# Nikhil-AI-Labs/image-super-resolution-2

Hardware: AMD Instinct MI355X
Metric: output MPix/s at x4 SR (256->1024) (higher is better)
Workload: dtype bf16 (bf16 MFMA operands, fp32 accumulate, fp32 activations in HBM)

## Files before the change

### image-super-resolution-2_amd/csrc/conv_gemm_bf16.hip

```cpp
#include "ff_common.h"

typedef __bf16 bf16x8 __attribute__((ext_vector_type(8)));
typedef __bf16 bf16x4 __attribute__((ext_vector_type(4)));

struct ConvBfParams {
  const float* in;
  const __bf16* w_hi;
  const __bf16* w_lo;
  const float* bias;
  const float* mul;
  const float* res;
  const float* kmul;
  float* out;
  int B, H, W, Cin, ldi;
  int Ho, Wo, Cout, ldo, ldr;
  int KH, KW, sy, sx, py, px;
  int K, Kp, M;
  int Cp;
  int act;
  float alpha;
  int shuffle;
  int vec_out;
  int gate;
};

template <int BM, int BN, int WM, int WN, bool VEC4, int NTERMS, int BKB>
__global__ __launch_bounds__(WM * WN * 64) void conv_igemm_bf16_kernel(ConvBfParams p) {
  constexpr int ROWB = BKB * 4 + 16, PLB = BKB * 2;
  constexpr int KQ = BKB / 4, QB = BKB / 8;
  constexpr int NT = WM * WN * 64;
  constexpr int TM = BM / WM, TN = BN / WN;
  constexpr int MI = TM / 32, NI = TN / 32;
  constexpr int RPP = NT / KQ;
  constexpr int AQ = BM / RPP;
  constexpr int BI = (BN * 2 * QB + NT - 1) / NT;
  static_assert(BM % RPP == 0, "A staging must tile the rows");
  extern __shared__ __attribute__((aligned(16))) unsigned char smem[];
  unsigned char* As = smem;
  unsigned char* Bs = smem + 2 * BM * ROWB;

  const int tid = threadIdx.x;
  const int lane = tid & 63, wid = tid >> 6;
  const int l31 = lane & 31, hh = lane >> 5;
  const int wr = wid / WN, wc = wid % WN;

  const int mtiles = (p.M + BM - 1) / BM, ntiles = (p.Cout + BN - 1) / BN;
  const int L = ff_xcd_remap(blockIdx.x, mtiles * ntiles);
  const int m0 = (L / ntiles) * BM, n0 = (L % ntiles) * BN;

  const int srow = tid / KQ, kq = tid % KQ;
  int a_b[AQ], a_iy[AQ], a_ix[AQ];
  bool a_ok[AQ];
#pragma unroll
  for (int i = 0; i < AQ; ++i) {
    const int m = m0 + srow + RPP * i;
    a_ok[i] = m < p.M;
    const int mm = a_ok[i] ? m : 0;
    const int ox = mm % p.Wo, t2 = mm / p.Wo;
    const int oy = t2 % p.Ho;
    a_b[i] = t2 / p.Ho;
    a_iy[i] = oy * p.sy - p.py;
    a_ix[i] = ox * p.sx - p.px;
  }
  const bool is1x1 = (p.KH == 1 && p.KW == 1);

  f32x4 ra[AQ];
  uint4 rb[BI];

  auto load_chunk = [&](int k0) {
    if (VEC4) {
      int ky = 0, kx = 0, ci;
      bool kok;
      if (p.Cp > 0) {
        const int tap = k0 / p.Cp;
        ci = k0 - tap * p.Cp + 4 * kq;
        kok = ci < p.Cin;
        ky = tap / p.KW;
        kx = tap - ky * p.KW;
      } else {
        const int k = k0 + 4 * kq;
        kok = k < p.K;
        ci = k;
        if (!is1x1 && kok) {
          const int tap = k / p.Cin;
          ci = k - tap * p.Cin;
          ky = tap / p.KW;
          kx = tap - ky * p.KW;
        }
      }
#pragma unroll
      for (int i = 0; i < AQ; ++i) {
        const int iy = a_iy[i] + ky, ix = a_ix[i] + kx;
        f32x4 v = {0.f, 0.f, 0.f, 0.f};
        if (kok && a_ok[i] && (unsigned)iy < (unsigned)p.H && (unsigned)ix < (unsigned)p.W)
          v = *reinterpret_cast<const f32x4*>(p.in + ((long long)(a_b[i] * p.H + iy) * p.W + ix) * p.ldi + ci);
        ra[i] = v;
      }
      if (p.kmul && kok) {
        const f32x4 km = *reinterpret_cast<const f32x4*>(p.kmul + ci);
#pragma unroll
        for (int i = 0; i < AQ; ++i) ra[i] *= km;
      }
    } else {
#pragma unroll
      for (int e = 0; e < 4; ++e) {
        const int k = k0 + 4 * kq + e;
        const bool kok = k < p.K;
        int ky = 0, kx = 0, ci = k;
// ... 17 lines not shown
    for (int j = 0; j < BI; ++j) {
      const int id = tid + NT * j;
      const int plane = id / (BN * QB), rem = id % (BN * QB);
      const int r = rem / QB, q = rem % QB;
      uint4 v = {0u, 0u, 0u, 0u};
      if (id < BN * 2 * QB && (NTERMS == 3 || plane == 0) && n0 + r < p.Cout) {
        const __bf16* src = (plane ? p.w_lo : p.w_hi) + (long long)(n0 + r) * p.Kp + k0 + 8 * q;
        v = *reinterpret_cast<const uint4*>(src);
      }
      rb[j] = v;
    }
  };

  auto store_chunk = [&](int buf) {
#pragma unroll
    for (int i = 0; i < AQ; ++i) {
      bf16x4 hi, lo;
#pragma unroll
      for (int e = 0; e < 4; ++e) {
        const float f = ra[i][e];
        const __bf16 h = (__bf16)f;
        hi[e] = h;
        lo[e] = (__bf16)(f - (float)h);
      }
      unsigned char* dst = As + (size_t)(buf * BM + srow + RPP * i) * ROWB + kq * 8;
      *reinterpret_cast<bf16x4*>(dst) = hi;
      if (NTERMS >= 2) *reinterpret_cast<bf16x4*>(dst + PLB) = lo;
    }
#pragma unroll
    for (int j = 0; j < BI; ++j) {
      const int id = tid + NT * j;
      const int plane = id / (BN * QB), rem = id % (BN * QB);
      const int r = rem / QB, q = rem % QB;
      if (id < BN * 2 * QB && (NTERMS == 3 || plane == 0))
        *reinterpret_cast<uint4*>(Bs + (size_t)(buf * BN + r) * ROWB + plane * PLB + q * 16) = rb[j];
    }
  };

  f32x16 acc[MI][NI];
#pragma unroll
  for (int i = 0; i < MI; ++i)
#pragma unroll
    for (int j = 0; j < NI; ++j)
#pragma unroll
      for (int r = 0; r < 16; ++r) acc[i][j][r] = 0.f;

  const int nchunks = p.Kp / BKB;
  load_chunk(0);
  store_chunk(0);
  __syncthreads();

  for (int c = 0; c < nchunks; ++c) {
    const int buf = c & 1;
    if (c + 1 < nchunks) load_chunk((c + 1) * BKB);
#pragma unroll
    for (int s = 0; s < BKB / 16; ++s) {
      bf16x8 ah[MI], al[MI], bh[NI], bl[NI];
#pragma unroll
      for (int i = 0; i < MI; ++i) {
        const unsigned char* ap = As + (size_t)(buf * BM + wr * TM + i * 32 + l31) * ROWB + 32 * s + 16 * hh;
        ah[i] = *reinterpret_cast<const bf16x8*>(ap);
        if (NTERMS >= 2) al[i] = *reinterpret_cast<const bf16x8*>(ap + PLB);
      }
#pragma unroll
      for (int j = 0; j < NI; ++j) {
        const unsigned char* bp = Bs + (size_t)(buf * BN + wc * TN + j * 32 + l31) * ROWB + 32 * s + 16 * hh;
        bh[j] = *reinterpret_cast<const bf16x8*>(bp);
        if (NTERMS == 3) bl[j] = *reinterpret_cast<const bf16x8*>(bp + PLB);
      }
#pragma unroll
      for (int i = 0; i < MI; ++i)
#pragma unroll
        for (int j = 0; j < NI; ++j) {
          if (NTERMS == 3) acc[i][j] = __builtin_amdgcn_mfma_f32_32x32x16_bf16(ah[i], bl[j], acc[i][j], 0, 0, 0);
          if (NTERMS >= 2) acc[i][j] = __builtin_amdgcn_mfma_f32_32x32x16_bf16(al[i], bh[j], acc[i][j], 0, 0, 0);
          acc[i][j] = __builtin_amdgcn_mfma_f32_32x32x16_bf16(ah[i], bh[j], acc[i][j], 0, 0, 0);
        }
    }
    if (c + 1 < nchunks) store_chunk(buf ^ 1);
    __syncthreads();
  }

  auto epilogue = [&](auto ACTC) {
    constexpr int ACT = decltype(ACTC)::value;
    const bool has_res = p.res != nullptr;
    if (p.gate) {
      float* tr = reinterpret_cast<float*>(smem) + wid * (32 * 36);
      const int grow = lane >> 2, seg = lane & 3;
#pragma unroll
      for (int j = 0; j < NI; ++j) {
        const int n = n0 + wc * TN + j * 32 + l31;
        const float bv = (p.bias && n < p.Cout) ? p.bias[n] : 0.f;
        const int nq = (n0 + wc * TN + j * 32) / 2 + 4 * seg;
        const bool nqok = nq < p.Cout / 2;
#pragma unroll
        for (int i = 0; i < MI; ++i) {
          const int mb = m0 + wr * TM + i * 32;
#pragma unroll
          for (int r = 0; r < 16; ++r) tr[((r & 3) + 8 * (r >> 2) + 4 * hh) * 36 + l31] = acc[i][j][r] + bv;
#pragma unroll
          for (int pass = 0; pass < 2; ++pass) {
            const int row = grow + 16 * pass;
            const f32x4 a = *reinterpret_cast<const f32x4*>(tr + row * 36 + 8 * seg);
            const f32x4 b2 = *reinterpret_cast<const f32x4*>(tr + row * 36 + 8 * seg + 4);
            const f32x4 o = {a[0] * a[1], a[2] * a[3], b2[0] * b2[1], b2[2] * b2[3]};
            const int m = mb + row;
            if (nqok && m < p.M) *reinterpret_cast<f32x4*>(p.out + (long long)m * p.ldo + nq) = o;
          }
        }
      }
      return;
    }
    if (p.vec_out) {
      float* tr = reinterpret_cast<float*>(smem) + wid * (32 * 36);
      const int tq = lane >> 3, q4 = 4 * (lane & 7);
#pragma unroll
      for (int j = 0; j < NI; ++j) {
        const int n = n0 + wc * TN + j * 32 + l31;
        const int nc = n < p.Cout ? n : 0;
        const float bv = p.bias ? p.bias[nc] : 0.f;
        const float mv = (p.mul ? p.mul[nc] : 1.f) * p.alpha;
        const int nq = n0 + wc * TN + j * 32 + q4;
        const bool nqok = nq < p.Cout;
#pragma unroll
        for (int i = 0; i < MI; ++i) {
          const int mb = m0 + wr * TM + i * 32;
          f32x4 rq[4];
          long long oo[4];
          bool ok[4];
#pragma unroll
          for (int k = 0; k < 4; ++k) {
            const int m = mb + tq + 8 * k;
            ok[k] = nqok && m < p.M;
            oo[k] = ok[k] ? (long long)m * p.ldo + nq : 0;
            f32x4 r0 = {0.f, 0.f, 0.f, 0.f};
            if (has_res) { const f32x4 u = *reinterpret_cast<const f32x4*>(p.res + (ok[k] ? (long long)m * p.ldr + nq : 0)); r0 = ok[k] ? u : r0; }
            rq[k] = r0;
          }
#pragma unroll
          for (int r = 0; r < 16; ++r)
            tr[((r & 3) + 8 * (r >> 2) + 4 * hh) * 36 + l31] = ff_act_c<ACT, true>(acc[i][j][r] + bv) * mv;
          f32x4 ov[4];
#pragma unroll
          for (int k = 0; k < 4; ++k) ov[k] = *reinterpret_cast<const f32x4*>(tr + (tq + 8 * k) * 36 + q4) + rq[k];
          if (nqok && mb + 32 <= p.M) {
#pragma unroll
            for (int k = 0; k < 4; ++k) *reinterpret_cast<f32x4*>(p.out + oo[k]) = ov[k];
          } else {
#pragma unroll
            for (int k = 0; k < 4; ++k)
              if (ok[k]) *reinterpret_cast<f32x4*>(p.out + oo[k]) = ov[k];
          }
        }
      }
      return;
    }
#pragma unroll
    for (int j = 0; j < NI; ++j) {
      const int n = n0 + wc * TN + j * 32 + l31;
      if (n >= p.Cout) continue;
      const float bv = p.bias ? p.bias[n] : 0.f;
      const float mv = (p.mul ? p.mul[n] : 1.f) * p.alpha;
#pragma unroll
      for (int i = 0; i < MI; ++i) {
        long long oidx[16];
        float rv[16];
        const int mb = m0 + wr * TM + i * 32 + 4 * hh;
        if (p.shuffle == 2) {
#pragma unroll
          for (int r = 0; r < 16; ++r) {
            const int m = mb + (r & 3) + 8 * (r >> 2);
            const int mm = m < p.M ? m : 0;
            const int ox = mm % p.Wo, t2 = mm / p.Wo;
            const int oy = t2 % p.Ho, b = t2 / p.Ho;
            const int co = n >> 2, dy = (n >> 1) & 1, dx = n & 1;
            const long long pix = ((long long)(b * 2 * p.Ho + 2 * oy + dy) * (2 * p.Wo) + 2 * ox + dx);
            oidx[r] = pix * p.ldo + co;
            rv[r] = has_res ? p.res[pix * p.ldr + co] : 0.f;
          }
        } else {
#pragma unroll
          for (int r = 0; r < 16; ++r) {
            const int m = mb + (r & 3) + 8 * (r >> 2);
            const int mm = m < p.M ? m : 0;
            oidx[r] = (long long)mm * p.ldo + n;
            rv[r] = has_res ? p.res[(long long)mm * p.ldr + n] : 0.f;
          }
        }
        if (mb + 28 < p.M) {
#pragma unroll
          for (int r = 0; r < 16; ++r) p.out[oidx[r]] = ff_act_c<ACT, true>(acc[i][j][r] + bv) * mv + rv[r];
        } else {
#pragma unroll
          for (int r = 0; r < 16; ++r) {
            const int m = mb + (r & 3) + 8 * (r >> 2);
            if (m < p.M) p.out[oidx[r]] = ff_act_c<ACT, true>(acc[i][j][r] + bv) * mv + rv[r];
          }
        }
      }
    }
  };
  FF_DISPATCH_ACT(p.act, epilogue)
}

template <int BM, int BN, int WM, int WN, int NT, int BKB = 32>
static int launch_bf(const ConvBfParams& p, bool vec4, hipStream_t st) {
  const int mt = ff_cdiv(p.M, BM), nt = ff_cdiv(p.Cout, BN);
  constexpr size_t lds = (size_t)2 * (BM + BN) * (BKB * 4 + 16);
  static_assert(lds <= 160 * 1024 && lds >= (size_t)WM * WN * 32 * 36 * 4, "LDS budget (staging ring; the epilogue patch reuses it)");
  dim3 grid((unsigned)(mt * nt)), block(WM * WN * 64);
  if (lds > 64 * 1024) {
    static bool attr_set[2] = {false, false};
    if (!attr_set[vec4 ? 1 : 0]) {
      hipError_t e = vec4 ? hipFuncSetAttribute(reinterpret_cast<const void*>(&conv_igemm_bf16_kernel<BM, BN, WM, WN, true, NT, BKB>),
                                                hipFuncAttributeMaxDynamicSharedMemorySize, (int)lds)
                          : hipFuncSetAttribute(reinterpret_cast<const void*>(&conv_igemm_bf16_kernel<BM, BN, WM, WN, false, NT, BKB>),
                                                hipFuncAttributeMaxDynamicSharedMemorySize, (int)lds);
      if (e != hipSuccess) { ff_set_error("ff_conv2d_bf16s: cannot raise dynamic LDS to %zu: %s", lds, hipGetErrorString(e)); return FF_ERR_LAUNCH; }
      attr_set[vec4 ? 1 : 0] = true;
    }
  }
  if (vec4)
    hipLaunchKernelGGL((conv_igemm_bf16_kernel<BM, BN, WM, WN, true, NT, BKB>), grid, block, lds, st, p);
  else
    hipLaunchKernelGGL((conv_igemm_bf16_kernel<BM, BN, WM, WN, false, NT, BKB>), grid, block, lds, st, p);
  FF_LAUNCH_CHECK("ff_conv2d_bf16s");
  return FF_OK;
}

template <int NT>
static int dispatch_bf(const ConvBfParams& p, bool vec4, int cfg, hipStream_t st) {
  switch (cfg) {
    case 1: return launch_bf<128, 128, 2, 2, NT>(p, vec4, st);
    case 2: return launch_bf<128, 64, 2, 2, NT>(p, vec4, st);
    case 3: return launch_bf<256, 32, 4, 1, NT>(p, vec4, st);
    case 4: return launch_bf<256, 192, 4, 2, NT>(p, vec4, st);
    case 5: return launch_bf<128, 128, 2, 4, NT>(p, vec4, st);
    case 6: return launch_bf<256, 128, 4, 2, NT>(p, vec4, st);
    case 7: return launch_bf<128, 64, 4, 2, NT>(p, vec4, st);
    case 8: return launch_bf<128, 128, 2, 4, NT, 64>(p, vec4, st);
    case 9: return launch_bf<128, 64, 4, 2, NT, 64>(p, vec4, st);
    default: ff_set_error("ff_conv2d_bf16s: bad tile_hint %d", cfg); return FF_ERR_ARG;
  }
}

extern "C" int ff_conv2d_bf16s(const float* in, const void* w_hi, const void* w_lo, int Kp, int Cp, const float* bias,
                               const float* mul, const float* res, float* out, int B, int H, int W, int Cin, int ldi,
                               int Ho, int Wo, int Cout, int ldo, int ldr, int KH, int KW, int sy, int sx, int py, int px,
                               int act, float alpha, int shuffle, int nterms, int tile_hint, const float* kmul, void* stream) {
  FF_CHECK_ARG(in && w_hi && out, "ff_conv2d_bf16s: null pointer");
  FF_CHECK_ARG(!kmul || (KH == 1 && KW == 1 && Cin % 4 == 0 && (((uintptr_t)kmul) & 15) == 0), "ff_conv2d_bf16s: kmul needs a 1x1 kernel, Cin %% 4 == 0 and a 16-byte aligned vector");
  FF_CHECK_ARG(nterms >= 1 && nterms <= 3 && (nterms < 3 || w_lo), "ff_conv2d_bf16s: nterms must be 1..3 (3 needs w_lo)");
  FF_CHECK_ARG(B > 0 && H > 0 && W > 0 && Cin > 0 && Cout > 0 && Ho > 0 && Wo > 0, "ff_conv2d_bf16s: bad dims");
  FF_CHECK_ARG(ldi >= Cin, "ff_conv2d_bf16s: ldi %d < Cin %d", ldi, Cin);
  FF_CHECK_ARG(KH > 0 && KW > 0 && sy > 0 && sx > 0 && py >= 0 && px >= 0, "ff_conv2d_bf16s: bad kernel geometry");
  FF_CHECK_ARG(Kp % 32 == 0 && Kp >= KH * KW * Cin, "ff_conv2d_bf16s: Kp must be K rounded up to 32");
  FF_CHECK_ARG(Cp == 0 || (Cp % 32 == 0 && Cp >= Cin && Kp == KH * KW * Cp), "ff_conv2d_bf16s: TAP layout needs Kp == taps * Cp, Cp = ceil32(Cin)");
  FF_CHECK_ARG((((uintptr_t)w_hi) & 15) == 0 && (!w_lo || (((uintptr_t)w_lo) & 15) == 0), "ff_conv2d_bf16s: weight planes must be 16-byte aligned");
  FF_CHECK_ARG(shuffle == 0 || shuffle == 1 || shuffle == 2, "ff_conv2d_bf16s: shuffle must be 0, 1 (SimpleGate pair product) or 2 (PixelShuffle)");
  FF_CHECK_ARG(shuffle != 2 || Cout % 4 == 0, "ff_conv2d_bf16s: shuffle needs Cout %% 4 == 0");
  FF_CHECK_ARG(shuffle != 1 || (Cout % 8 == 0 && !res && !mul && act == 0 && alpha == 1.f && ldo % 4 == 0 && (((uintptr_t)out) & 15) == 0),
               "ff_conv2d_bf16s: the pair-product epilogue needs Cout %% 8 == 0, no residual / scale / activation and 16-byte aligned output rows");
  FF_CHECK_ARG(ldo >= (shuffle == 2 ? Cout / 4 : shuffle == 1 ? Cout / 2 : Cout), "ff_conv2d_bf16s: ldo too small");
  FF_CHECK_ARG(!res || ldr >= (shuffle ? Cout / 4 : Cout), "ff_conv2d_bf16s: ldr too small");
  FF_CHECK_ARG((long long)B * Ho * Wo < (1LL << 31), "ff_conv2d_bf16s: M overflows int");
  ConvBfParams p;
  p.in = in; p.w_hi = (const __bf16*)w_hi; p.w_lo = (const __bf16*)w_lo; p.bias = bias; p.mul = mul; p.res = res; p.out = out;
  p.kmul = kmul; p.gate = shuffle == 1 ? 1 : 0;
  p.B = B; p.H = H; p.W = W; p.Cin = Cin; p.ldi = ldi;
  p.Ho = Ho; p.Wo = Wo; p.Cout = Cout; p.ldo = ldo; p.ldr = ldr;
  p.KH = KH; p.KW = KW; p.sy = sy; p.sx = sx; p.py = py; p.px = px;
  p.K = KH * KW * Cin; p.Kp = Kp; p.Cp = Cp; p.M = B * Ho * Wo;
  p.act = act; p.alpha = alpha; p.shuffle = shuffle;
  p.vec_out = shuffle == 0 && Cout % 4 == 0 && ldo % 4 == 0 && (((uintptr_t)out) & 15) == 0 &&
              (!res || (ldr % 4 == 0 && (((uintptr_t)res) & 15) == 0));
  const bool vec4 = (Cin % 4 == 0) && (ldi % 4 == 0) && (((uintptr_t)in & 15) == 0);
  FF_CHECK_ARG(Cp == 0 || vec4, "ff_conv2d_bf16s: TAP layout needs Cin %% 4 == 0 and 16-byte aligned rows");
  FF_CHECK_ARG(!kmul || vec4, "ff_conv2d_bf16s: kmul needs 16-byte aligned input rows");
  hipStream_t st = (hipStream_t)stream;
  int cfg = tile_hint;
  if (cfg <= 0) {
    const int r192 = Cout % 192, r128 = Cout % 128;
    if (Cout <= 32) cfg = 3;
    else if (Cout <= 64) cfg = 7;
    else if (r128 == 0) cfg = 5;
    else if (vec4 && p.M >= 256 * 64 && (r192 == 0 || r192 > 128) && (Cout <= 192 || p.K >= 320)) cfg = 4;
    else if (Cout > 256 || (Cout > 128 && p.K >= 512)) cfg = 5;
    else cfg = 7;
  }
  const bool k64 = Kp % 64 == 0 && (Cp == 0 || Cp % 64 == 0) && vec4;
  if (cfg >= 8 && !k64) cfg = cfg == 8 ? 5 : 7;
  switch (nterms) {
    case 1: return dispatch_bf<1>(p, vec4, cfg, st);
    case 2: return dispatch_bf<2>(p, vec4, cfg, st);
    default: return dispatch_bf<3>(p, vec4, cfg, st);
  }
}

__global__ __launch_bounds__(256) void split_bf16_kernel(const float* __restrict__ w, int N, int K, int Kp, int Cin, int Cp,
                                                         __bf16* __restrict__ hi, __bf16* __restrict__ lo) {
  const long long total = (long long)N * Kp;
  for (long long i = (long long)blockIdx.x * 256 + threadIdx.x; i < total; i += (long long)gridDim.x * 256) {
    const int kp = (int)(i % Kp);
    const long long n = i / Kp;
    int k = kp;
    bool ok = kp < K;
    if (Cp > 0) { const int tap = kp / Cp, ci = kp - tap * Cp; ok = ci < Cin; k = tap * Cin + ci; }
    const float f = ok ? w[n * K + k] : 0.f;
    const __bf16 h = (__bf16)f;
    hi[i] = h;
    if (lo) lo[i] = (__bf16)(f - (float)h);
  }
}

extern "C" int ff_split_bf16(const float* w, int N, int K, int Kp, int Cin, int Cp, void* hi, void* lo, void* stream) {
  FF_CHECK_ARG(w && hi && N > 0 && K > 0 && Kp % 32 == 0 && Kp >= K, "ff_split_bf16: bad args");
  FF_CHECK_ARG(Cp == 0 || (Cin > 0 && K % Cin == 0 && Cp % 32 == 0 && Cp >= Cin && Kp == (K / Cin) * Cp), "ff_split_bf16: bad TAP layout");
  long long nb = ((long long)N * Kp + 255) / 256;
  if (nb > 4096) nb = 4096;
  hipLaunchKernelGGL(split_bf16_kernel, dim3((unsigned)nb), dim3(256), 0, (hipStream_t)stream, w, N, K, Kp, Cin, Cp, (__bf16*)hi, (__bf16*)lo);
  FF_LAUNCH_CHECK("ff_split_bf16");
  return FF_OK;
}
```

### image-super-resolution-2_amd/ops.py

```python
from __future__ import annotations

from typing import Dict, Optional, Tuple

import torch

from . import lib as _lib

ACT = {None: 0, "none": 0, "gelu": 1, "relu": 2, "lrelu": 3, "sigmoid": 4}
T = torch.Tensor

_PROF = None
_META = [0.0, 0.0]


def _note(flops: float = 0.0, nbytes: float = 0.0):
    _META[0] += flops
    _META[1] += nbytes


def _numel(*ts) -> float:
    return float(sum(t.numel() * (t.element_size() / 4.0) for t in ts if t is not None))


def _instrument(fn):
# ... 297 lines not shown
    elif tuple(out.shape) != oshape:
        raise _lib.FFError(f"conv2d: out shape {tuple(out.shape)} != {oshape}")
    out_bf16 = out.dtype == torch.bfloat16
    op, ldo, *_ = _nhwc(out, "conv2d.out|bf16ok" if out_bf16 else "conv2d.out")
    halo_ok = (_HALO and _GEMM_MODE in ("bf16x3", "bf16") and (KH, KW) == (3, 3) and tuple(stride) == (1, 1) and tuple(pad) == (1, 1)
               and not dynamic_w and Cin >= 32 and Cin % 4 == 0 and ldi % 4 == 0 and xp % 16 == 0
               and (Cout <= 64 or Cin >= 128 or 128 < Cout <= 192 or _HALO_ALL) and H * W >= 1024 and xp != op and B * H * W * ldi < 2 ** 31)
    if (in_bf16 or out_bf16) and not (halo_ok and _GEMM_MODE == "bf16" and shuffle == 0 and res is None):
        raise _lib.FFError("conv2d: bf16 input / output rows exist for the LDS-resident 3x3 kernel in plain-bf16 mode only")
    rp, ldr = None, 0
    if res is not None:
        if tuple(res.shape) != oshape:
            raise _lib.FFError(f"conv2d: res shape {tuple(res.shape)} != {oshape}")
        rp, ldr, *_ = _nhwc(res, "conv2d.res")
    if (_SMALL and _GEMM_MODE != "f32" and (KH, KW) == (3, 3) and tuple(stride) == (1, 1) and tuple(pad) == (1, 1) and Cout <= 16
            and Cin * (1 if Cout == 1 else (4 if Cout <= 4 else 16)) <= 128 and shuffle == 0 and mul is None and not dynamic_w and H * W >= 4096 and xp != op):
        from . import prep as _prep
        ws = PREPARED.get(w, "small", lambda: _prep.pack_conv3x3_small(w, Cin))
        _lib.check(_L().ff_conv3x3_small(xp, ldi, ws.data_ptr(), ws.shape[2], _ptr(bias), rp, ldr, op, ldo, B, H, W, Cin, Cout, ACT[act],
                                         float(alpha), _stream()))
    elif _GEMM_MODE == "f32":
        _lib.check(_L().ff_conv2d(xp, w.data_ptr(), _ptr(bias), _ptr(mul), rp, op, B, H, W, Cin, ldi, Ho, Wo, Cout, ldo, ldr,
                                  KH, KW, stride[0], stride[1], pad[0], pad[1], ACT[act], float(alpha), shuffle, tile_hint,
                                  _stream()))
    elif (_HALO and _GEMM_MODE in ("bf16x3", "bf16") and (KH, KW) == (3, 3) and tuple(stride) == (1, 1) and tuple(pad) == (1, 1)
          and not dynamic_w and Cin >= 32 and Cin % 4 == 0 and ldi % 4 == 0 and xp % 16 == 0
          and (Cout <= 64 or Cin >= 128 or 128 < Cout <= 192 or _HALO_ALL)
          and H * W >= 1024 and xp != op and B * H * W * ldi < 2 ** 31):
        from . import prep as _prep

        nt_ = _nterms()

        def _mk_halo():
            bn = _prep.halo_bn(Cout)
            return (_prep.pack_conv3x3_halo(w, Cin, bn, nt_), bn)
        img = PREPARED.get(w, "halo" if nt_ == 3 else "halo1", _mk_halo)
        part = None
        if want_pool and B == 1 and shuffle == 0 and Cout <= img[1]:
            prow = int(_L().ff_conv3x3_halo_pool_rows(B, H, W, Cout, img[1], nt_))
            part = torch.empty((prow, img[1]), device=x.device, dtype=torch.float32)
        _lib.check(_L().ff_conv3x3_halo(xp, ldi, img[0].data_ptr(), img[1], _ptr(bias), _ptr(mul), rp, ldr, op, ldo, B, H, W,
                                        Cin, Cout, ACT[act], float(alpha), shuffle, _ptr(part), _nterms(),
                                        (1 if in_bf16 else 0) | (2 if out_bf16 else 0), _stream()))
        if part is not None:
            pp = PoolPartials(part, Cout, 1.0 / float(H * W))
            _note(2.0 * B * Ho * Wo * Cout * KH * KW * Cin, 4.0 * (_numel(x, w, out, res)))
            return out, (pp if want_pool == "partials" else pp.mean())
    else:
        aligned = (ldi % 4 == 0) and (xp % 16 == 0)
        hi, lo, Kp, Cp, _ = _split_weight(w, dynamic_w, Cin if aligned else 0)
        _lib.check(_L().ff_conv2d_bf16s(xp, hi.data_ptr(), lo.data_ptr() if lo is not None else None, Kp, Cp, _ptr(bias), _ptr(mul),
                                        rp, op, B, H, W, Cin, ldi, Ho, Wo, Cout, ldo, ldr, KH, KW, stride[0], stride[1],
                                        pad[0], pad[1], ACT[act], float(alpha), shuffle, GEMM_MODES[_GEMM_MODE], tile_hint,
                                        None, _stream()))
    _note(2.0 * B * Ho * Wo * Cout * KH * KW * Cin, 4.0 * (_numel(x, w, out, res)))
    if want_pool:
        return out, pool_mean(out)
    return out


def cab_fused(x: T, w1: T, b1: T, w2: T, b2: T, partials: bool = False):
    if _GEMM_MODE != "bf16":
        raise _lib.FFError("cab_fused exists for the plain-bf16 contraction mode only")
    xp, ldi, B, H, W, Cin = _nhwc(x, "cab_fused.x")
    Cmid, Cout = w1.shape[0], w2.shape[0]
    if B != 1 or w1.shape[1] != 9 * Cin or w2.shape[1] != 9 * Cmid:
        raise _lib.FFError("cab_fused: expects one image and packed 3x3 weights [Cmid, 9*Cin], [Cout, 9*Cmid]")
    from . import prep as _prep
    i1 = PREPARED.get(w1, "cab1", lambda: _prep.pack_conv3x3_halo(w1, Cin, 64, 1))
    i2 = PREPARED.get(w2, "cab2", lambda: _prep.pack_conv3x3_halo(w2, Cmid, 192, 1))
    out = empty_rows((1, H, W, Cout), x.device)
    op, ldo, *_ = _nhwc(out, "cab_fused.out")
    prow = int(_L().ff_cab_fused_pool_rows(H, W))
    part = torch.empty((prow, 192), device=x.device, dtype=torch.float32)
    _lib.check(_L().ff_cab_fused(xp, ldi, i1.data_ptr(), b1.data_ptr(), i2.data_ptr(), b2.data_ptr(), op, ldo, H, W, Cin, Cmid, Cout,
                                 part.data_ptr(), _stream()))
    pp = PoolPartials(part, Cout, 1.0 / float(H * W))
    _note(2.0 * H * W * 9 * (Cmid * Cin + Cout * Cmid), 4.0 * H * W * (Cin + Cout))
    return out, (pp if partials else pp.mean())


def linear(x: T, w: T, bias: Optional[T] = None, *, act=None, res: Optional[T] = None, mul: Optional[T] = None,
           alpha: float = 1.0, out: Optional[T] = None, dynamic_w: bool = False, kmul: Optional[T] = None,
           gate_pairs: bool = False) -> T:
    xp, ldi, rows, K = rows_view(x, "linear.x")
    N = w.shape[0]
    if w.dim() != 2 or w.shape[1] != K or not w.is_contiguous():
        raise _lib.FFError(f"linear: weight must be [N, {K}], got {tuple(w.shape)}")
    if (kmul is not None or gate_pairs) and _GEMM_MODE == "f32":
        raise _lib.FFError("linear: kmul / gate_pairs exist in the split-bf16 kernels only")
    No = N // 2 if gate_pairs else N
    oshape = tuple(x.shape[:-1]) + (No,)
    if out is None:
        out = empty_rows(oshape, x.device)
    op, ldo, orows, oc = rows_view(out, "linear.out")
    if orows != rows or oc != No:
        raise _lib.FFError("linear: out shape mismatch")
    rp, ldr = None, 0
    if res is not None:
        rp, ldr, rrows, rc = rows_view(res, "linear.res")
        if rrows != rows or rc != N:
            raise _lib.FFError("linear: res shape mismatch")
    if _GEMM_MODE == "f32":
        _lib.check(_L().ff_conv2d(xp, w.data_ptr(), _ptr(bias), _ptr(mul), rp, op, 1, 1, rows, K, ldi, 1, rows, N, ldo, ldr,
                                  1, 1, 1, 1, 0, 0, ACT[act], float(alpha), 0, 0, _stream()))
    else:
        aligned = (ldi % 4 == 0) and (xp % 16 == 0)
        hi, lo, Kp, Cp, _ = _split_weight(w, dynamic_w, K if aligned else 0)
        if kmul is not None and (kmul.numel() != K or not kmul.is_contiguous()):
            raise _lib.FFError(f"linear: kmul must be a contiguous [{K}] vector")
        _lib.check(_L().ff_conv2d_bf16s(xp, hi.data_ptr(), lo.data_ptr() if lo is not None else None, Kp, Cp, _ptr(bias), _ptr(mul),
                                        rp, op, 1, 1, rows, K, ldi, 1, rows, N, ldo, ldr, 1, 1, 1, 1, 0, 0, ACT[act],
                                        float(alpha), 1 if gate_pairs else 0, GEMM_MODES[_GEMM_MODE], 0, _ptr(kmul), _stream()))
    _note(2.0 * rows * N * K, 4.0 * (rows * K + N * K + rows * No * (2 if res is not None else 1)))
    return out


def window_attn(qkv: T, out: T, biasT: T, *, q_off: int, k_off: int, v_off: int, o_off: int, H: int, W: int, Hp: int,
                Wp: int, win: Tuple[int, int], kwin: Tuple[int, int], shift: Tuple[int, int], use_mask: bool, heads: int,
                d: int, scale: float, rel_table: Optional[T] = None) -> T:
    qp, ldq, B, h_, w_, _ = _nhwc(qkv, "window_attn.qkv")
    op, ldo, *_ = _nhwc(out, "window_attn.out")
    if (h_, w_) != (H, W) or tuple(out.shape[:3]) != (B, H, W):
        raise _lib.FFError("window_attn: qkv/out spatial dims mismatch")
    nk = kwin[0] * kwin[1]
    if tuple(biasT.shape) != (heads, nk, 256) or not biasT.is_contiguous():
        raise _lib.FFError(f"window_attn: biasT must be [{heads},{nk},256]")
    if q_off + heads * d > qkv.shape[-1] or k_off + heads * d > qkv.shape[-1] or v_off + heads * d > qkv.shape[-1] \
            or o_off + heads * d > out.shape[-1]:
        raise _lib.FFError("window_attn: channel offsets out of range")
    if _GEMM_MODE == "f32":
        _lib.check(_L().ff_window_attn(qp, ldq, q_off, k_off, v_off, op, ldo, o_off, biasT.data_ptr(), B, H, W, Hp, Wp, win[0],
                                       win[1], kwin[0], kwin[1], shift[0], shift[1], int(use_mask), heads, d, float(scale),
                                       _stream()))
    else:
        relp = None
        if rel_table is not None and tuple(kwin) != tuple(win):
            n = (win[0] + kwin[0] - 1) * (win[1] + kwin[1] - 1)
            if tuple(rel_table.shape) != (heads, n) or not rel_table.is_contiguous() or kwin[1] % 8 or tuple(shift) != (0, 0):
                raise _lib.FFError(f"window_attn: overlapping-window rel_table must be [heads, {n}] (prep.pack_rel_overlap), kw % 8 == 0, no shift")
            relp = rel_table.data_ptr()
        elif rel_table is not None and tuple(kwin) == tuple(win) and win[1] & (win[1] - 1) == 0 and win[1] >= 8:
            if tuple(rel_table.shape) != (heads, (2 * win[0] - 1) * (2 * win[1] - 1)) or not rel_table.is_contiguous():
                raise _lib.FFError("window_attn: rel_table must be [heads, (2wh-1)*(2ww-1)]")
            relp = rel_table.data_ptr()
        from . import prep as _prep
        bq = PREPARED.get(biasT, "quad", lambda: _prep.quad_bias(biasT))
        _lib.check(_L().ff_window_attn_bf16s(qp, ldq, q_off, k_off, v_off, op, ldo, o_off, bq.data_ptr(), B, H, W, Hp, Wp,
                                             win[0], win[1], kwin[0], kwin[1], shift[0], shift[1], int(use_mask), heads, d,
                                             float(scale), 1 if _GEMM_MODE == "bf16" else 3, relp, _stream()))
    nwin = B * (Hp // win[0]) * (Wp // win[1])
    _note(4.0 * nwin * heads * 256 * nk * d, 4.0 * (4.0 * B * H * W * heads * d + heads * nk * 256))
    return out


def ocab_attn(qkv: T, out: T, rel_rotated: T, *, q_off: int, k_off: int, v_off: int, o_off: int = 0, H: int, W: int, heads: int, d: int,
              ws: int, ows: int, scale: float) -> T:
    if _GEMM_MODE != "bf16":
        raise _lib.FFError("ocab_attn exists for the plain-bf16 contraction mode only")
    qp, ldq, B, h_, w_, _ = _nhwc(qkv, "ocab_attn.qkv")
    out_bf16 = out.dtype == torch.bfloat16
    op, ldo, *_ = _nhwc(out, "ocab_attn.out|bf16ok" if out_bf16 else "ocab_attn.out")
    if (h_, w_) != (H, W) or tuple(out.shape[:3]) != (B, H, W) or tuple(rel_rotated.shape) != (heads, (ws + ows - 1) ** 2) or not rel_rotated.is_contiguous():
        raise _lib.FFError("ocab_attn: shape mismatch")
    _lib.check(_L().ff_ocab_attn(qp, ldq, q_off, k_off, v_off, op, ldo, o_off, rel_rotated.data_ptr(), B, H, W, heads, d, ws, ows,
                                 float(scale), int(out_bf16), _stream()))
    nwin = B * (H // ws) * (W // ws)
    _note(4.0 * nwin * heads * ws * ws * ows * ows * d, 4.0 * B * H * W * heads * d * 4)
    return out


def win_attn_fused(x: T, out: T, pk: dict, rel_padded: T, *, gamma: Optional[T], beta: Optional[T], eps: float = 1e-5,
                   H: int, W: int, Hp: int, Wp: int, win: Tuple[int, int], shift: Tuple[int, int], use_mask: bool,
                   head0: int = 0, nheads: Optional[int] = None, o_off: int = 0, zero_pad: bool = False,
                   want_xn: bool = False, v_out: Optional[T] = None, v_off: int = 0):
    xp, ldx, B, h_, w_, K = _nhwc(x, "win_attn_fused.x")
    out_bf16 = out.dtype == torch.bfloat16
    op, ldo, *_ = _nhwc(out, "win_attn_fused.out|bf16ok" if out_bf16 else "win_attn_fused.out")
    xn_bf16 = want_xn == "bf16"
    if (out_bf16 or xn_bf16) and _GEMM_MODE != "bf16":
        raise _lib.FFError("win_attn_fused: bf16 outputs exist for the plain-bf16 contraction mode only")
    if (h_, w_) != (H, W) or tuple(out.shape[:3]) != (B, H, W) or K != pk["K"]:
        raise _lib.FFError("win_attn_fused: x/out dims mismatch")
    nheads = pk["heads"] - head0 if nheads is None else nheads
    if tuple(rel_padded.shape[:2]) != (pk["heads"], 2 * win[0] - 1) or not rel_padded.is_contiguous():
        raise _lib.FFError("win_attn_fused: rel_padded must be [heads][2wh-1][stride]")
    if _GEMM_MODE not in ("bf16x3", "bf16"):
        raise _lib.FFError("win_attn_fused exists for the bf16 contraction modes only")
    xn, xnp, ldxn = None, None, 0
    if want_xn:
        xn = empty_rows_bf16(tuple(x.shape), x.device) if xn_bf16 else empty_like_rows(x)
        xnp, ldxn, _, _ = rows_view(xn, "win_attn_fused.xn|bf16ok" if xn_bf16 else "win_attn_fused.xn")
    vp, ldv = None, 0
    if v_out is not None:
        vp, ldv, vb, vh, vw, _ = _nhwc(v_out, "win_attn_fused.v_out")
        if (vb, vh, vw) != (B, H, W):
# ... 553 lines not shown
```

Baseline: 24.25.

## Add multi-stage async-LDS pipelined bf16 kernel for 1x1 convolutions and linears

```diff
diff --git a/image-super-resolution-2_amd/csrc/conv_gemm_bf16.hip b/image-super-resolution-2_amd/csrc/conv_gemm_bf16.hip
--- a/image-super-resolution-2_amd/csrc/conv_gemm_bf16.hip
+++ b/image-super-resolution-2_amd/csrc/conv_gemm_bf16.hip
@@ -1,4 +1,6 @@
 #include "ff_common.h"
+
+extern "C" int ff_device_cu_count(void);
 
 typedef __bf16 bf16x8 __attribute__((ext_vector_type(8)));
 typedef __bf16 bf16x4 __attribute__((ext_vector_type(4)));
@@ -24,6 +26,126 @@
   int gate;
 };
 
+template <int ACT, int MI, int NI, int TM, int TN>
+__device__ __forceinline__ void bf_epilogue(const ConvBfParams& p, f32x16 (&acc)[MI][NI], float* tr, int m0, int n0, int wr, int wc,
+                                            int lane) {
+  const int l31 = lane & 31, hh = lane >> 5;
+  const bool has_res = p.res != nullptr;
+  if (p.gate) {
+    const int grow = lane >> 2, seg = lane & 3;
+#pragma unroll
+    for (int j = 0; j < NI; ++j) {
+      const int n = n0 + wc * TN + j * 32 + l31;
+      const float bv = (p.bias && n < p.Cout) ? p.bias[n] : 0.f;
+      const int nq = (n0 + wc * TN + j * 32) / 2 + 4 * seg;
+      const bool nqok = nq < p.Cout / 2;
+#pragma unroll
+      for (int i = 0; i < MI; ++i) {
+        const int mb = m0 + wr * TM + i * 32;
+#pragma unroll
+        for (int r = 0; r < 16; ++r) tr[((r & 3) + 8 * (r >> 2) + 4 * hh) * 36 + l31] = acc[i][j][r] + bv;
+#pragma unroll
+        for (int pass = 0; pass < 2; ++pass) {
+          const int row = grow + 16 * pass;
+          const f32x4 a = *reinterpret_cast<const f32x4*>(tr + row * 36 + 8 * seg);
+          const f32x4 b2 = *reinterpret_cast<const f32x4*>(tr + row * 36 + 8 * seg + 4);
+          const f32x4 o = {a[0] * a[1], a[2] * a[3], b2[0] * b2[1], b2[2] * b2[3]};
+          const int m = mb + row;
+          if (nqok && m < p.M) *reinterpret_cast<f32x4*>(p.out + (long long)m * p.ldo + nq) = o;
+        }
+      }
+    }
+    return;
+  }
+  if (p.vec_out) {
+    const int tq = lane >> 3, q4 = 4 * (lane & 7);
+#pragma unroll
+    for (int j = 0; j < NI; ++j) {
+      const int n = n0 + wc * TN + j * 32 + l31;
+      const int nc = n < p.Cout ? n : 0;
+      const float bv = p.bias ? p.bias[nc] : 0.f;
+      const float mv = (p.mul ? p.mul[nc] : 1.f) * p.alpha;
+      const int nq = n0 + wc * TN + j * 32 + q4;
+      const bool nqok = nq < p.Cout;
+#pragma unroll
+      for (int i = 0; i < MI; ++i) {
+        const int mb = m0 + wr * TM + i * 32;
+        f32x4 rq[4];
+        long long oo[4];
+        bool ok[4];
+#pragma unroll
+        for (int k = 0; k < 4; ++k) {
+          const int m = mb + tq + 8 * k;
+          ok[k] = nqok && m < p.M;
+          oo[k] = ok[k] ? (long long)m * p.ldo + nq : 0;
+          f32x4 r0 = {0.f, 0.f, 0.f, 0.f};
+          if (has_res) { const f32x4 u = *reinterpret_cast<const f32x4*>(p.res + (ok[k] ? (long long)m * p.ldr + nq : 0)); r0 = ok[k] ? u : r0; }
+          rq[k] = r0;
+        }
+#pragma unroll
+        for (int r = 0; r < 16; ++r)
+          tr[((r & 3) + 8 * (r >> 2) + 4 * hh) * 36 + l31] = ff_act_c<ACT, true>(acc[i][j][r] + bv) * mv;
+        f32x4 ov[4];
+#pragma unroll
+        for (int k = 0; k < 4; ++k) ov[k] = *reinterpret_cast<const f32x4*>(tr + (tq + 8 * k) * 36 + q4) + rq[k];
+        if (nqok && mb + 32 <= p.M) {
+#pragma unroll
+          for (int k = 0; k < 4; ++k) *reinterpret_cast<f32x4*>(p.out + oo[k]) = ov[k];
+        } else {
+#pragma unroll
+          for (int k = 0; k < 4; ++k)
+            if (ok[k]) *reinterpret_cast<f32x4*>(p.out + oo[k]) = ov[k];
+        }
+      }
+    }
+    return;
+  }
+#pragma unroll
+  for (int j = 0; j < NI; ++j) {
+    const int n = n0 + wc * TN + j * 32 + l31;
+    if (n >= p.Cout) continue;
+    const float bv = p.bias ? p.bias[n] : 0.f;
+    const float mv = (p.mul ? p.mul[n] : 1.f) * p.alpha;
+#pragma unroll
+    for (int i = 0; i < MI; ++i) {
+      long long oidx[16];
+      float rv[16];
+      const int mb = m0 + wr * TM + i * 32 + 4 * hh;
+      if (p.shuffle == 2) {
+#pragma unroll
+        for (int r = 0; r < 16; ++r) {
+          const int m = mb + (r & 3) + 8 * (r >> 2);
+          const int mm = m < p.M ? m : 0;
+          const int ox = mm % p.Wo, t2 = mm / p.Wo;
+          const int oy = t2 % p.Ho, b = t2 / p.Ho;
+          const int co = n >> 2, dy = (n >> 1) & 1, dx = n & 1;
+          const long long pix = ((long long)(b * 2 * p.Ho + 2 * oy + dy) * (2 * p.Wo) + 2 * ox + dx);
+          oidx[r] = pix * p.ldo + co;
+          rv[r] = has_res ? p.res[pix * p.ldr + co] : 0.f;
+        }
+      } else {
+#pragma unroll
+        for (int r = 0; r < 16; ++r) {
+          const int m = mb + (r & 3) + 8 * (r >> 2);
+          const int mm = m < p.M ? m : 0;
+          oidx[r] = (long long)mm * p.ldo + n;
+          rv[r] = has_res ? p.res[(long long)mm * p.ldr + n] : 0.f;
+        }
+      }
+      if (mb + 28 < p.M) {
+#pragma unroll
+        for (int r = 0; r < 16; ++r) p.out[oidx[r]] = ff_act_c<ACT, true>(acc[i][j][r] + bv) * mv + rv[r];
+      } else {
+#pragma unroll
+        for (int r = 0; r < 16; ++r) {
+          const int m = mb + (r & 3) + 8 * (r >> 2);
+          if (m < p.M) p.out[oidx[r]] = ff_act_c<ACT, true>(acc[i][j][r] + bv) * mv + rv[r];
+        }
+      }
+    }
+  }
+}
+
 template <int BM, int BN, int WM, int WN, bool VEC4, int NTERMS, int BKB>
 __global__ __launch_bounds__(WM * WN * 64) void conv_igemm_bf16_kernel(ConvBfParams p) {
   constexpr int ROWB = BKB * 4 + 16, PLB = BKB * 2;
@@ -207,125 +329,163 @@
   }
 
   auto epilogue = [&](auto ACTC) {
-    constexpr int ACT = decltype(ACTC)::value;
-    const bool has_res = p.res != nullptr;
-    if (p.gate) {
-      float* tr = reinterpret_cast<float*>(smem) + wid * (32 * 36);
-      const int grow = lane >> 2, seg = lane & 3;
-#pragma unroll
-      for (int j = 0; j < NI; ++j) {
-        const int n = n0 + wc * TN + j * 32 + l31;
-        const float bv = (p.bias && n < p.Cout) ? p.bias[n] : 0.f;
-        const int nq = (n0 + wc * TN + j * 32) / 2 + 4 * seg;
-        const bool nqok = nq < p.Cout / 2;
-#pragma unroll
-        for (int i = 0; i < MI; ++i) {
-          const int mb = m0 + wr * TM + i * 32;
-#pragma unroll
-          for (int r = 0; r < 16; ++r) tr[((r & 3) + 8 * (r >> 2) + 4 * hh) * 36 + l31] = acc[i][j][r] + bv;
-#pragma unroll
-          for (int pass = 0; pass < 2; ++pass) {
-            const int row = grow + 16 * pass;
-            const f32x4 a = *reinterpret_cast<const f32x4*>(tr + row * 36 + 8 * seg);
-            const f32x4 b2 = *reinterpret_cast<const f32x4*>(tr + row * 36 + 8 * seg + 4);
-            const f32x4 o = {a[0] * a[1], a[2] * a[3], b2[0] * b2[1], b2[2] * b2[3]};
-            const int m = mb + row;
-            if (nqok && m < p.M) *reinterpret_cast<f32x4*>(p.out + (long long)m * p.ldo + nq) = o;
-          }
-        }
-      }
-      return;
-    }
-    if (p.vec_out) {
-      float* tr = reinterpret_cast<float*>(smem) + wid * (32 * 36);
-      const int tq = lane >> 3, q4 = 4 * (lane & 7);
-#pragma unroll
-      for (int j = 0; j < NI; ++j) {
-        const int n = n0 + wc * TN + j * 32 + l31;
-        const int nc = n < p.Cout ? n : 0;
-        const float bv = p.bias ? p.bias[nc] : 0.f;
-        const float mv = (p.mul ? p.mul[nc] : 1.f) * p.alpha;
-        const int nq = n0 + wc * TN + j * 32 + q4;
-        const bool nqok = nq < p.Cout;
-#pragma unroll
-        for (int i = 0; i < MI; ++i) {
-          const int mb = m0 + wr * TM + i * 32;
-          f32x4 rq[4];
-          long long oo[4];
-          bool ok[4];
-#pragma unroll
-          for (int k = 0; k < 4; ++k) {
-            const int m = mb + tq + 8 * k;
-            ok[k] = nqok && m < p.M;
-            oo[k] = ok[k] ? (long long)m * p.ldo + nq : 0;
-            f32x4 r0 = {0.f, 0.f, 0.f, 0.f};
-            if (has_res) { const f32x4 u = *reinterpret_cast<const f32x4*>(p.res + (ok[k] ? (long long)m * p.ldr + nq : 0)); r0 = ok[k] ? u : r0; }
-            rq[k] = r0;
-          }
-#pragma unroll
-          for (int r = 0; r < 16; ++r)
-            tr[((r & 3) + 8 * (r >> 2) + 4 * hh) * 36 + l31] = ff_act_c<ACT, true>(acc[i][j][r] + bv) * mv;
-          f32x4 ov[4];
-#pragma unroll
-          for (int k = 0; k < 4; ++k) ov[k] = *reinterpret_cast<const f32x4*>(tr + (tq + 8 * k) * 36 + q4) + rq[k];
-          if (nqok && mb + 32 <= p.M) {
-#pragma unroll
-            for (int k = 0; k < 4; ++k) *reinterpret_cast<f32x4*>(p.out + oo[k]) = ov[k];
-          } else {
-#pragma unroll
-            for (int k = 0; k < 4; ++k)
-              if (ok[k]) *reinterpret_cast<f32x4*>(p.out + oo[k]) = ov[k];
-          }
-        }
-      }
-      return;
-    }
-#pragma unroll
-    for (int j = 0; j < NI; ++j) {
-      const int n = n0 + wc * TN + j * 32 + l31;
-      if (n >= p.Cout) continue;
-      const float bv = p.bias ? p.bias[n] : 0.f;
-      const float mv = (p.mul ? p.mul[n] : 1.f) * p.alpha;
-#pragma unroll
-      for (int i = 0; i < MI; ++i) {
-        long long oidx[16];
-        float rv[16];
-        const int mb = m0 + wr * TM + i * 32 + 4 * hh;
-        if (p.shuffle == 2) {
-#pragma unroll
-          for (int r = 0; r < 16; ++r) {
-            const int m = mb + (r & 3) + 8 * (r >> 2);
-            const int mm = m < p.M ? m : 0;
-            const int ox = mm % p.Wo, t2 = mm / p.Wo;
-            const int oy = t2 % p.Ho, b = t2 / p.Ho;
-            const int co = n >> 2, dy = (n >> 1) & 1, dx = n & 1;
-            const long long pix = ((long long)(b * 2 * p.Ho + 2 * oy + dy) * (2 * p.Wo) + 2 * ox + dx);
-            oidx[r] = pix * p.ldo + co;
-            rv[r] = has_res ? p.res[pix * p.ldr + co] : 0.f;
-          }
-        } else {
-#pragma unroll
-          for (int r = 0; r < 16; ++r) {
-            const int m = mb + (r & 3) + 8 * (r >> 2);
-            const int mm = m < p.M ? m : 0;
-            oidx[r] = (long long)mm * p.ldo + n;
-            rv[r] = has_res ? p.res[(long long)mm * p.ldr + n] : 0.f;
-          }
-        }
-        if (mb + 28 < p.M) {
-#pragma unroll
-          for (int r = 0; r < 16; ++r) p.out[oidx[r]] = ff_act_c<ACT, true>(acc[i][j][r] + bv) * mv + rv[r];
-        } else {
-#pragma unroll
-          for (int r = 0; r < 16; ++r) {
-            const int m = mb + (r & 3) + 8 * (r >> 2);
-            if (m < p.M) p.out[oidx[r]] = ff_act_c<ACT, true>(acc[i][j][r] + bv) * mv + rv[r];
-          }
-        }
-      }
-    }
+    bf_epilogue<decltype(ACTC)::value, MI, NI, TM, TN>(p, acc, reinterpret_cast<float*>(smem) + wid * (32 * 36), m0, n0, wr, wc, lane);
   };
   FF_DISPATCH_ACT(p.act, epilogue)
+}
+
+namespace pipe1x1 {
+constexpr int BM = 128, BN = 128, BK = 32, NW = 4, WN = 2;
+constexpr int ASLOT = BM * BK * 4, BSLOT = BN * BK * 2, SLOT = ASLOT + BSLOT;
+constexpr int APC = ASLOT / 1024 / NW, BPC = BSLOT / 1024 / NW;
+constexpr int KMUL_MAX = 1024;
+constexpr size_t lds(int nslot) { return (size_t)nslot * SLOT + KMUL_MAX * 4; }
+static_assert(APC + BPC == 6, "wait_ahead counts 6 pieces per wave and chunk");
+static_assert(NW * 32 * 36 * 4 <= SLOT, "epilogue patches fit in one ring slot");
+static_assert(2 * lds(3) <= 160 * 1024 && lds(6) <= 160 * 1024, "3 slots: two workgroups per CU; 6 slots: one");
+__device__ __forceinline__ void wait_ahead(int ahead) {
+  switch (ahead) {
+    case 0: asm volatile("s_waitcnt vmcnt(0)" ::: "memory"); break;
+    case 1: asm volatile("s_waitcnt vmcnt(6)" ::: "memory"); break;
+    case 2: asm volatile("s_waitcnt vmcnt(12)" ::: "memory"); break;
+    case 3: asm volatile("s_waitcnt vmcnt(18)" ::: "memory"); break;
+    default: asm volatile("s_waitcnt vmcnt(24)" ::: "memory"); break;
+  }
+}
+}
+
+template <bool KMUL, int NSLOT>
+__global__ __launch_bounds__(pipe1x1::NW * 64, NSLOT <= 3 ? 2 : 1) void conv_igemm_bf16_pipe1x1_kernel(ConvBfParams p) {
+  using namespace pipe1x1;
+  static_assert(NSLOT >= 3 && NSLOT <= 6, "ring of 3 .. 6 slots");
+  constexpr int DEPTH = NSLOT - 1;
+  constexpr int TM = BM / (NW / WN), TN = BN / WN, MI = TM / 32, NI = TN / 32;
+  extern __shared__ __attribute__((aligned(16))) unsigned char smem[];
+  float* kms = reinterpret_cast<float*>(smem + NSLOT * SLOT);
+
+  const int tid = threadIdx.x, lane = tid & 63, wid = tid >> 6;
+  const int l31 = lane & 31, hh = lane >> 5;
+  const int wr = wid / WN, wc = wid % WN;
+  const int mtiles = (p.M + BM - 1) / BM, ntiles = (p.Cout + BN - 1) / BN;
+  const int L = ff_xcd_remap(blockIdx.x, mtiles * ntiles);
+  const int m0 = (L / ntiles) * BM, n0 = (L % ntiles) * BN;
+
+  if (KMUL) {
+    for (int k = 4 * tid; k < p.Kp; k += 4 * NW * 64)
+      *reinterpret_cast<f32x4*>(kms + k) = *reinterpret_cast<const f32x4*>(p.kmul + k);
+  }
+
+  const float* asrc[APC];
+  const __bf16* bsrc[BPC];
+#pragma unroll
+  for (int i = 0; i < APC; ++i) {
+    const int r = 8 * (wid + NW * i) + (lane >> 3);
+    const int m = min(m0 + r, p.M - 1);
+    asrc[i] = p.in + (long long)m * p.ldi + 4 * ((lane & 7) ^ ((r >> 1) & 7));
+  }
+#pragma unroll
+  for (int i = 0; i < BPC; ++i) {
+    const int r = 16 * (wid + NW * i) + (lane >> 2);
+    const int n = min(n0 + r, p.Cout - 1);
+    bsrc[i] = p.w_hi + (long long)n * p.Kp + 8 * ((lane & 3) ^ ((r >> 2) & 3));
+  }
+  auto dma = [&](int c, int slot) {
+    const int k0 = c * BK;
+    unsigned char* as = smem + slot * SLOT;
+    unsigned char* bs = as + ASLOT;
+#pragma unroll
+    for (int i = 0; i < APC; ++i)
+      __builtin_amdgcn_global_load_lds((const __attribute__((address_space(1))) void*)(asrc[i] + k0),
+                                       (__attribute__((address_space(3))) void*)(as + (wid + NW * i) * 1024), 16, 0, 0);
+#pragma unroll
+    for (int i = 0; i < BPC; ++i)
+      __builtin_amdgcn_global_load_lds((const __attribute__((address_space(1))) void*)(bsrc[i] + k0),
+                                       (__attribute__((address_space(3))) void*)(bs + (wid + NW * i) * 1024), 16, 0, 0);
+  };
+
+  const int xa = (l31 >> 1) & 7, xb = (l31 >> 2) & 3;
+  int aoff[MI], boff[NI];
+#pragma unroll
+  for (int i = 0; i < MI; ++i) aoff[i] = (wr * TM + i * 32 + l31) * (BK * 4);
+#pragma unroll
+  for (int j = 0; j < NI; ++j) boff[j] = ASLOT + (wc * TN + j * 32 + l31) * (BK * 2);
+
+  f32x16 acc[MI][NI];
+#pragma unroll
+  for (int i = 0; i < MI; ++i)
+#pragma unroll
+    for (int j = 0; j < NI; ++j)
+#pragma unroll
+      for (int r = 0; r < 16; ++r) acc[i][j][r] = 0.f;
+
+  const int nchunks = p.Kp / BK;
+#pragma unroll
+  for (int d = 0; d < DEPTH; ++d)
+    if (d < nchunks) dma(d, d);
+  for (int c = 0; c < nchunks; ++c) {
+    wait_ahead(min(DEPTH - 1, nchunks - 1 - c));
+    asm volatile("s_waitcnt lgkmcnt(0)" ::: "memory");
+    __builtin_amdgcn_s_barrier();
+    if (c + DEPTH < nchunks) dma(c + DEPTH, (c + DEPTH) % NSLOT);
+    const unsigned char* slot = smem + (c % NSLOT) * SLOT;
+    constexpr int KS = BK / 16;
+    f32x4 ua[KS][MI][2], km[KS][2];
+    bf16x8 bh[KS][NI];
+#pragma unroll
+    for (int s = 0; s < KS; ++s) {
+      const int ga = 4 * s + 2 * hh, gb = 2 * s + hh;
+#pragma unroll
+      for (int i = 0; i < MI; ++i) {
+        ua[s][i][0] = *reinterpret_cast<const f32x4*>(slot + aoff[i] + 16 * (ga ^ xa));
+        ua[s][i][1] = *reinterpret_cast<const f32x4*>(slot + aoff[i] + 16 * ((ga + 1) ^ xa));
+      }
+#pragma unroll
+      for (int j = 0; j < NI; ++j) bh[s][j] = *reinterpret_cast<const bf16x8*>(slot + boff[j] + 16 * (gb ^ xb));
+      if (KMUL) {
+        km[s][0] = *reinterpret_cast<const f32x4*>(kms + c * BK + 16 * s + 8 * hh);
+        km[s][1] = *reinterpret_cast<const f32x4*>(kms + c * BK + 16 * s + 8 * hh + 4);
+      }
+    }
+#pragma unroll
+    for (int s = 0; s < KS; ++s) {
+      bf16x8 ah[MI];
+#pragma unroll
+      for (int i = 0; i < MI; ++i) {
+        f32x4 u0 = ua[s][i][0], u1 = ua[s][i][1];
+        if (KMUL) { u0 *= km[s][0]; u1 *= km[s][1]; }
+#pragma unroll
+        for (int e = 0; e < 4; ++e) {
+          ah[i][e] = (__bf16)u0[e];
+          ah[i][4 + e] = (__bf16)u1[e];
+        }
+      }
+#pragma unroll
+      for (int i = 0; i < MI; ++i)
+#pragma unroll
+        for (int j = 0; j < NI; ++j) acc[i][j] = __builtin_amdgcn_mfma_f32_32x32x16_bf16(ah[i], bh[s][j], acc[i][j], 0, 0, 0);
+    }
+  }
+
+  float* tr = reinterpret_cast<float*>(smem + ((nchunks + NSLOT - 2) % NSLOT) * SLOT) + wid * (32 * 36);
+  auto epilogue = [&](auto ACTC) { bf_epilogue<decltype(ACTC)::value, MI, NI, TM, TN>(p, acc, tr, m0, n0, wr, wc, lane); };
+  FF_DISPATCH_ACT(p.act, epilogue)
+}
+
+template <bool KMUL, int NSLOT>
+static int launch_pipe1x1(const ConvBfParams& p, hipStream_t st) {
+  using namespace pipe1x1;
+  constexpr size_t LDS = lds(NSLOT);
+  static bool attr_set = false;
+  if (!attr_set) {
+    hipError_t e = hipFuncSetAttribute(reinterpret_cast<const void*>(&conv_igemm_bf16_pipe1x1_kernel<KMUL, NSLOT>),
+                                       hipFuncAttributeMaxDynamicSharedMemorySize, (int)LDS);
+    if (e != hipSuccess) { ff_set_error("ff_conv2d_bf16s: cannot raise dynamic LDS to %zu: %s", LDS, hipGetErrorString(e)); return FF_ERR_LAUNCH; }
+    attr_set = true;
+  }
+  dim3 grid((unsigned)(ff_cdiv(p.M, BM) * ff_cdiv(p.Cout, BN))), block(NW * 64);
+  hipLaunchKernelGGL((conv_igemm_bf16_pipe1x1_kernel<KMUL, NSLOT>), grid, block, LDS, st, p);
+  FF_LAUNCH_CHECK("ff_conv2d_bf16s");
+  return FF_OK;
 }
 
 template <int BM, int BN, int WM, int WN, int NT, int BKB = 32>
@@ -413,6 +573,20 @@
     else if (Cout > 256 || (Cout > 128 && p.K >= 512)) cfg = 5;
     else cfg = 7;
   }
+  const bool pipe_ok = nterms == 1 && vec4 && KH == 1 && KW == 1 && sy == 1 && sx == 1 && py == 0 && px == 0 && Ho == H && Wo == W &&
+                       Cin % 32 == 0 && Kp == Cin && (!kmul || Kp <= pipe1x1::KMUL_MAX);
+  if (tile_hint <= 0 && pipe_ok && cfg == 5 && Kp >= 256) {
+    static int ncu = 0;
+    if (ncu <= 0) ncu = ff_device_cu_count();
+    const long long tiles = (long long)ff_cdiv(p.M, pipe1x1::BM) * ff_cdiv(Cout, pipe1x1::BN);
+    cfg = (ncu > 0 && tiles <= ncu) ? 11 : 10;
+  }
+  if (cfg == 10 || cfg == 11) {
+    FF_CHECK_ARG(pipe_ok, "ff_conv2d_bf16s: tile_hint %d needs nterms == 1, a 1x1 / stride-1 kernel, Cin %% 32 == 0, 16-byte aligned input rows "
+                          "and Cin <= %d with kmul", cfg, pipe1x1::KMUL_MAX);
+    if (cfg == 10) return kmul ? launch_pipe1x1<true, 3>(p, st) : launch_pipe1x1<false, 3>(p, st);
+    return kmul ? launch_pipe1x1<true, 6>(p, st) : launch_pipe1x1<false, 6>(p, st);
+  }
   const bool k64 = Kp % 64 == 0 && (Cp == 0 || Cp % 64 == 0) && vec4;
   if (cfg >= 8 && !k64) cfg = cfg == 8 ? 5 : 7;
   switch (nterms) {
diff --git a/image-super-resolution-2_amd/ops.py b/image-super-resolution-2_amd/ops.py
--- a/image-super-resolution-2_amd/ops.py
+++ b/image-super-resolution-2_amd/ops.py
@@ -403,7 +403,7 @@
 
 def linear(x: T, w: T, bias: Optional[T] = None, *, act=None, res: Optional[T] = None, mul: Optional[T] = None,
            alpha: float = 1.0, out: Optional[T] = None, dynamic_w: bool = False, kmul: Optional[T] = None,
-           gate_pairs: bool = False) -> T:
+           gate_pairs: bool = False, tile_hint: int = 0) -> T:
     xp, ldi, rows, K = rows_view(x, "linear.x")
     N = w.shape[0]
     if w.dim() != 2 or w.shape[1] != K or not w.is_contiguous():
@@ -424,7 +424,7 @@
             raise _lib.FFError("linear: res shape mismatch")
     if _GEMM_MODE == "f32":
         _lib.check(_L().ff_conv2d(xp, w.data_ptr(), _ptr(bias), _ptr(mul), rp, op, 1, 1, rows, K, ldi, 1, rows, N, ldo, ldr,
-                                  1, 1, 1, 1, 0, 0, ACT[act], float(alpha), 0, 0, _stream()))
+                                  1, 1, 1, 1, 0, 0, ACT[act], float(alpha), 0, tile_hint, _stream()))
     else:
         aligned = (ldi % 4 == 0) and (xp % 16 == 0)
         hi, lo, Kp, Cp, _ = _split_weight(w, dynamic_w, K if aligned else 0)
@@ -432,7 +432,7 @@
             raise _lib.FFError(f"linear: kmul must be a contiguous [{K}] vector")
         _lib.check(_L().ff_conv2d_bf16s(xp, hi.data_ptr(), lo.data_ptr() if lo is not None else None, Kp, Cp, _ptr(bias), _ptr(mul),
                                         rp, op, 1, 1, rows, K, ldi, 1, rows, N, ldo, ldr, 1, 1, 1, 1, 0, 0, ACT[act],
-                                        float(alpha), 1 if gate_pairs else 0, GEMM_MODES[_GEMM_MODE], 0, _ptr(kmul), _stream()))
+                                        float(alpha), 1 if gate_pairs else 0, GEMM_MODES[_GEMM_MODE], tile_hint, _ptr(kmul), _stream()))
     _note(2.0 * rows * N * K, 4.0 * (rows * K + N * K + rows * No * (2 if res is not None else 1)))
     return out
 
```

After: 24.60 (median of 6 runs). 1.5% higher.
